# esulimma/LONER

Measured on AMD Instinct MI355X. Metric: ray-samples/sec per optimizer step; rendered-depth L1 vs reference, higher is better.
Workload: dtype fp16 params/activations, fp32 accumulate+optimizer; 1 GPU; C2: 16 KF x (512 + 0 sky) rays x 512 samples per GPU, L=16 T=2^18 hash grid + 64-wide sigma MLP, default loss (L1_JS); rays_per_gpu=8192, samples_per_ray=512, global_rays=8192, parallelism=single, optimizer=replicated, launch=HIP graph replay (one graph per window and OGM-or-not step), field_state=trained: the steps below follow 384 untimed pre-training steps (config.pretrain), poses=fixed (ground-truth poses, use_gt_poses: the north-star driver)

## Files before the change

### include/loner_amd.h

```cpp
#ifndef LONER_AMD_H
#define LONER_AMD_H

#include <stdint.h>

#ifdef __cplusplus
extern "C" {
#endif

#define LNR_OK 0
#define LNR_ERR_ARG (-1)
#define LNR_ERR_HIP (-2)

#define LNR_MAX_LEVELS 32

const char* lnr_last_error(void);
int lnr_version(void);

typedef struct lnr_step_scalars {
  uint32_t key;
  float los_lambda;
  float los_eps;
  float adam_step_size;
  float adam_bc2_sqrt;
  uint32_t pad[3];
// ... 147 lines not shown

int lnr_composite(const float* rays, const float* z, const float* sigma, int64_t n_rays, int32_t n_samples,
                  int32_t strategy, float noise_std, const float* noise, uint32_t key, int64_t ray_offset,
                  float* weights, float* depth, float* opacity, float* variance, void* stream);
int lnr_composite_loss_bwd(const float* rays, const float* z, const float* sigma, const float* depth_gt,
                           int64_t n_rays, int32_t n_samples, float noise_std, const float* noise, uint32_t key,
                           int64_t ray_offset, const lnr_loss_params* lp, float* weights, float* depth,
                           float* opacity, float* d_sigma, float* ray_stats, void* stream);
int lnr_composite_bwd(const float* rays, const float* z, const float* sigma, int64_t n_rays, int32_t n_samples,
                      int32_t strategy, float noise_std, const float* noise, uint32_t key, int64_t ray_offset,
                      const float* g_weights, const float* g_depth, const float* g_opacity, const float* g_variance,
                      float* d_sigma, float* d_ray, void* stream);
int64_t lnr_field_train_workspace_words(int64_t n_rays, int32_t n_samples);
int lnr_field_train(const uint16_t* w, const uint32_t* enc, int64_t enc_stride, const float* rays, const float* z,
                    const float* depth_gt, int64_t n_rays, int32_t n_samples, float noise_std, const float* noise,
                    uint32_t key, int64_t ray_offset, const lnr_loss_params* lp, float* d_enc, float* d_w,
                    float* workspace, float* ray_stats, float* depth, float* opacity, float* weights,
                    float* d_enc_level_max, uint32_t* d_enc_jac, void* stream);
int lnr_field_sigma_phase(const uint16_t* w, const uint32_t* enc, int64_t enc_stride, const float* rays,
                          const float* z, int64_t n_rays, int32_t n_samples, int32_t lo, int32_t hi, float noise_std,
                          const float* noise, uint32_t key, int64_t ray_offset, const lnr_loss_params* lp,
                          float* workspace, const uint32_t* list_in, const uint32_t* count_in, uint32_t* list_out,
                          uint32_t* count_out, double* transmittance, void* scratch, void* stream);
int lnr_pose_grad(const float* rays, const float* z, const float* d_pos, const float* d_ray, int64_t n_rays,
                  int32_t n_samples, const int64_t* slots, int64_t slot0, const int32_t* slot_kf, const float* slot_pose,
                  const float* pose6, int32_t n_kf, float scale, float far_range, float* ray_ws, float* grad,
                  void* stream);
int lnr_pose_adam(float* pose6, float* m, float* v, const float* grad, const uint8_t* optimise, int32_t n_kf,
                  int64_t step, float lr, float beta1, float beta2, float eps, float* rows, void* stream);
int lnr_field_render(const uint16_t* w, const uint32_t* enc, int64_t enc_stride, const float* rays, const float* z,
                     int64_t n_rays, int32_t n_samples, int32_t strategy, float noise_std, const float* noise,
                     uint32_t key, int64_t ray_offset, float* depth, float* opacity, float* variance,
                     float* weights, void* stream);
int lnr_rgb_render(const uint16_t* w_rgb, int32_t n_hidden_layers, const uint32_t* enc_rgb, int64_t enc_stride,
                   const float* rays, const float* weights, int64_t n_rays, int32_t n_samples, float* rgb,
                   void* stream);
int lnr_loss_finalize(const float* ray_stats, int64_t n_rays, const lnr_loss_params* lp, float* out, void* stream);

int lnr_count_opaque(const float* depth_gt, int64_t n_rays, float far_ref, const float* dev_far_ref, float* out,
                     void* stream);

#define LNR_SELECT_RANDOM 0
#define LNR_SELECT_MASK 1
#define LNR_SELECT_ALL 2
#define LNR_SELECT_GIVEN 3

// ... 113 lines not shown
```

### loner_amd/_lib.py

```python
import ctypes
import os

import torch

LIB_PATH = os.path.join(os.path.dirname(os.path.abspath(__file__)), "_lib", "libloner_amd.so")
LIB_PATH = os.environ.get("LONER_AMD_LIB", LIB_PATH)
MAX_LEVELS = 32
RAY_STATS = 5
SIGMA_MLP_PARAMS = 64 * 32 + 16 * 64

LOSS_KINDS = {"L1_JS": 0, "L2_JS": 1, "L1_LOS": 2, "L2_LOS": 3}
RENDER_STRATEGIES = {"default": 0, "adjusted": 1}
BWD_COUNTS_READY = 1
BWD_NO_ACCUM = 2
BWD_LEVEL_MAX_READY = 4
BWD_LIVE = 8
BWD_PREPARE_ONLY = 16
BWD_PREPARED = 32

c_p = ctypes.c_void_p
c_i64 = ctypes.c_int64
c_i32 = ctypes.c_int32
c_u32 = ctypes.c_uint32
c_f = ctypes.c_float
# ... 21 lines not shown
ADAM_MAX_RANGES = 8


class AdamEpilogue(ctypes.Structure):
    _fields_ = [("param", ctypes.c_void_p), ("shadow", ctypes.c_void_p), ("m", ctypes.c_void_p), ("v", ctypes.c_void_p),
                ("step", ctypes.c_int32), ("lr", ctypes.c_double), ("beta1", ctypes.c_double),
                ("beta2", ctypes.c_double), ("eps", ctypes.c_double), ("dev_step", ctypes.c_void_p)]


class LossParams(ctypes.Structure):
    _fields_ = [("kind", ctypes.c_int32), ("scale", ctypes.c_float), ("los_lambda", ctypes.c_float),
                ("depthloss_lambda", ctypes.c_float), ("min_depth_eps", ctypes.c_float),
                ("min_js", ctypes.c_float), ("max_js", ctypes.c_float), ("js_alpha", ctypes.c_float),
                ("los_eps", ctypes.c_float), ("far_ref", ctypes.c_float), ("inv_n_opaque", ctypes.c_float),
                ("inv_rs", ctypes.c_float), ("dev_n_opaque", ctypes.c_void_p), ("dev_far_ref", ctypes.c_void_p),
                ("dev_status", ctypes.c_void_p), ("dev_loss_out", ctypes.c_void_p), ("flags", ctypes.c_int32),
                ("dev_step", ctypes.c_void_p), ("dev_d_ray", ctypes.c_void_p), ("dev_term_hist", ctypes.c_void_p)]


LP_DW_OVERWRITE = 1
LP_SIGMA_READY = 2
LP_FORWARD_ONLY = 4
LP_BACKWARD_ONLY = 8


STATUS_NAN_LOSS, STATUS_INF_LOSS, STATUS_SIGMA_CLIPPED, STATUS_NONFINITE_OUTPUT = 1, 2, 4, 8


SELECT = {"RANDOM": 0, "MASK": 1, "ALL": 2, "GIVEN": 3}


class RayWindowDesc(ctypes.Structure):
    _fields_ = [("n_kf", ctypes.c_int32), ("scale", ctypes.c_float), ("shift", ctypes.c_float * 3),
                ("r_min", ctypes.c_float), ("r_max", ctypes.c_float), ("poses", c_p), ("dirs", c_p), ("dists", c_p),
                ("scan_off", c_p), ("order", c_p), ("n_trunk", c_p), ("sky_dirs", c_p), ("sky_off", c_p),
                ("ray_off", c_p), ("n_sel", c_p), ("n_sel_trunk", c_p), ("dev_step", c_p)]


class MotionComp(ctypes.Structure):
    _fields_ = [("start_rot", ctypes.c_float * 9), ("start_t", ctypes.c_float * 3), ("delta_t", ctypes.c_float * 3),
                ("axis", ctypes.c_float * 3), ("angle", ctypes.c_float), ("t0", ctypes.c_float), ("t1", ctypes.c_float),
                ("target_inv", ctypes.c_float * 12), ("identity", ctypes.c_int32)]


class CameraDesc(ctypes.Structure):
    _fields_ = [("width", ctypes.c_int32), ("height", ctypes.c_int32), ("channels", ctypes.c_int32),
# ... 34 lines not shown
    "lnr_hashgrid_bwd_rays_atomic": (ctypes.c_int, [ctypes.POINTER(GridDesc), c_p, c_p, c_i64, c_i32, c_p, c_i64, c_p,
                                                    c_p]),
    "lnr_enc_to_aos": (ctypes.c_int, [c_p, c_i64, c_i64, c_u32, c_p, c_p]),
    "lnr_aos_grad_to_enc": (ctypes.c_int, [c_p, c_p, c_i64, c_u32, c_p, c_i64, c_p]),
    "lnr_sh_encode": (ctypes.c_int, [c_p, c_i64, c_i32, c_p, c_p]),
    "lnr_sigma_mlp_fwd": (ctypes.c_int, [c_p, c_p, c_i64, c_i64, c_p, c_p]),
    "lnr_dw_workspace_words": (c_i64, [c_i64]),
    "lnr_field_train_workspace_words": (c_i64, [c_i64, c_i32]),
    "lnr_sigma_mlp_bwd": (ctypes.c_int, [c_p, c_p, c_i64, c_i64, c_p, c_p, c_p, c_p, c_p]),
    "lnr_step_key": (c_u32, [c_u32, c_u32]),
    "lnr_sample_ogm": (ctypes.c_int, [c_p, c_i64, c_i32, c_p, c_i32, c_f, c_p, c_p, c_u32, c_i64, c_p, c_p, c_p]),
    "lnr_sample_uniform": (ctypes.c_int, [c_p, c_i64, c_i32, c_f, c_p, c_u32, c_i64, c_p, c_p, c_p]),
    "lnr_composite": (ctypes.c_int, [c_p, c_p, c_p, c_i64, c_i32, c_i32, c_f, c_p, c_u32, c_i64, c_p, c_p, c_p, c_p,
                                     c_p]),
    "lnr_composite_bwd": (ctypes.c_int, [c_p, c_p, c_p, c_i64, c_i32, c_i32, c_f, c_p, c_u32, c_i64, c_p, c_p, c_p,
                                         c_p, c_p, c_p, c_p]),
    "lnr_composite_loss_bwd": (ctypes.c_int, [c_p, c_p, c_p, c_p, c_i64, c_i32, c_f, c_p, c_u32, c_i64,
                                              ctypes.POINTER(LossParams), c_p, c_p, c_p, c_p, c_p, c_p]),
    "lnr_field_train": (ctypes.c_int, [c_p, c_p, c_i64, c_p, c_p, c_p, c_i64, c_i32, c_f, c_p, c_u32, c_i64,
                                       ctypes.POINTER(LossParams), c_p, c_p, c_p, c_p, c_p, c_p, c_p, c_p, c_p,
                                       c_p]),
    "lnr_field_sigma_phase": (ctypes.c_int, [c_p, c_p, c_i64, c_p, c_p, c_i64, c_i32, c_i32, c_i32, c_f, c_p, c_u32,
                                             c_i64, ctypes.POINTER(LossParams), c_p, c_p, c_p, c_p, c_p, c_p, c_p, c_p]),
    "lnr_pose_grad": (ctypes.c_int, [c_p, c_p, c_p, c_p, c_i64, c_i32, c_p, c_i64, c_p, c_p, c_p, c_i32, c_f, c_f, c_p,
                                     c_p, c_p]),
    "lnr_pose_adam": (ctypes.c_int, [c_p, c_p, c_p, c_p, c_p, c_i32, c_i64, c_f, c_f, c_f, c_f, c_p, c_p]),
    "lnr_field_render": (ctypes.c_int, [c_p, c_p, c_i64, c_p, c_p, c_i64, c_i32, c_i32, c_f, c_p, c_u32, c_i64, c_p,
                                        c_p, c_p, c_p, c_p]),
    "lnr_rgb_render": (ctypes.c_int, [c_p, c_i32, c_p, c_i64, c_p, c_p, c_i64, c_i32, c_p, c_p]),
    "lnr_hashgrid_fwd_rays_phase": (ctypes.c_int, [ctypes.POINTER(GridDesc), c_p, c_p, c_i64, c_i32, c_p, c_p, c_i64,
                                                   c_p, c_i64, c_p, c_p, c_i64, c_i32, c_i32, c_p]),
    "lnr_hashgrid_fwd_rays_live": (ctypes.c_int, [ctypes.POINTER(GridDesc), c_p, c_p, c_i64, c_i32, c_p, c_p, c_p, c_i64,
                                                  c_p]),
    "lnr_hashgrid_fwd_rays_live_ws": (ctypes.c_int, [ctypes.POINTER(GridDesc), c_p, c_p, c_i64, c_i32, c_p, c_p, c_p,
                                                     c_i64, c_p, c_i64, c_p]),
    "lnr_hashgrid_bwd_rays_live": (ctypes.c_int, [ctypes.POINTER(GridDesc), c_p, c_p, c_i64, c_i32, c_p, c_i64, c_p, c_p,
                                                  c_p, c_i64, c_i32, c_p]),
    "lnr_status_scan": (ctypes.c_int, [c_p, c_i64, c_u32, c_p, c_p]),
    "lnr_rgb_mlp_params": (c_i64, [c_i32]),
    "lnr_rgb_train_workspace_bytes": (c_i64, [c_i32, c_i64]),
    "lnr_rgb_train": (ctypes.c_int, [c_p, c_i32, c_p, c_i64, c_p, c_p, c_p, c_i64, c_i32, c_f, c_p, c_p, c_p, c_p,
                                     c_p, c_i64, c_p, c_p]),
    "lnr_build_camera_rays": (ctypes.c_int, [ctypes.POINTER(CameraDesc), c_p, c_p, c_p, c_i64, c_p, c_p, c_p]),
    "lnr_build_camera_rays_window": (ctypes.c_int, [c_p, c_i32, c_p, c_p, c_i64, c_i64, c_i64, c_p, c_p, c_p]),
    "lnr_motion_compensate": (ctypes.c_int, [ctypes.POINTER(MotionComp), c_p, c_p, c_p, c_i64, c_p]),
    "lnr_sky_rays_capacity": (c_i64, []),
# ... 83 lines not shown
```

### loner_amd/csrc/field.hip

```cpp
#include "common.hpp"
#include "mlp.hpp"

namespace lnr {

constexpr int NT = 256;
constexpr int NW = NT / 64;

enum SigmaSrc { kSigmaGiven = 0, kSigmaMLP = 1 };

struct FieldArgs {
  const float* rays;
  const float* z;
  const float* sigma_in;
  const uint16_t* w;
  const uint32_t* enc;
  int64_t enc_stride;
  const float* depth_gt;
  const float* noise;
  int64_t n_rays;
  int32_t S;
  float noise_std;
  uint32_t key;
  int64_t ray_offset;
  lnr_loss_params lp;
// ... 845 lines not shown
#pragma unroll
    for (int j = 0; j < kErtCompactPer; ++j) mine += r[j] != ~0u ? 1u : 0u;
    uint32_t inc = mine;
#pragma unroll
    for (int o = 1; o < 64; o <<= 1) {
      const uint32_t v = __shfl_up(inc, o, 64);
      if (lane >= o) inc += v;
    }
    if (lane == 63) wsum[wid] = inc;
    __syncthreads();
    uint32_t off = base + inc - mine, tot = 0;
    for (int w = 0; w < kErtCompactThreads / 64; ++w) {
      const uint32_t v = wsum[w];
      if (w < wid) off += v;
      tot += v;
    }
#pragma unroll
    for (int j = 0; j < kErtCompactPer; ++j)
      if (r[j] != ~0u) list_out[off++] = r[j];
    base += tot;
    __syncthreads();
  }
  if (t == 0) count_out[0] = base;
}

template <int C>
__global__ void __launch_bounds__(NT) k_composite_wave(FieldArgs a) {
  if (a.denc_max && blockIdx.x == 0 && threadIdx.x < kSigmaLevels) a.denc_max[threadIdx.x] = 0.f;
  extern __shared__ __attribute__((aligned(16))) char smem[];
  const int lane = threadIdx.x & 63, wid = threadIdx.x >> 6;
  constexpr int S = 64 * C;
  float* sig = reinterpret_cast<float*>(smem) + wid * S;
  for (int64_t r = (int64_t)blockIdx.x * kWavesPerBlock + wid; r < a.n_rays; r += (int64_t)gridDim.x * kWavesPerBlock) {
#pragma unroll
    for (int k = 0; k < C; ++k) sig[64 * k + lane] = a.d_sigma[r * S + 64 * k + lane];
    wave_lds_handoff();
    composite_loss_wave<C>(a, sig, r);
    wave_lds_handoff();
#pragma unroll
    for (int k = 0; k < C; ++k) a.d_sigma[r * S + 64 * k + lane] = sig[64 * k + lane];
    wave_lds_handoff();
  }
}

template <class T>
__device__ __forceinline__ T ld_off(const T* base, uint32_t byte_off) {
// ... 687 lines not shown
  LNR_REQUIRE(n_rays < (int64_t(1) << 31), "lnr_field_sigma_phase: too many rays");
  if (n_rays == 0) return LNR_OK;
  LNR_REQUIRE(w && enc && workspace && (lo == 0 || (list_in && count_in)) && (!list_in || count_in),
              "lnr_field_sigma_phase: null pointer (a phase after the first needs the list of rays still alive)");
  LNR_REQUIRE(hi == n_samples || (list_out && count_out && transmittance && scratch),
              "lnr_field_sigma_phase: null pointer (the phase's transmittance update)");
  FieldArgs a{};
  a.w = w; a.enc = enc; a.enc_stride = enc_stride; a.rays = rays; a.z = z; a.n_rays = n_rays; a.S = n_samples;
  a.noise_std = noise_std; a.noise = noise; a.key = key; a.ray_offset = ray_offset;
  if (lp) a.lp = *lp;
  a.d_sigma = workspace + lnr_dw_workspace_words(n_rays);
  hipStream_t st = as_stream(stream);
  const uint32_t* lin = lo == 0 ? nullptr : list_in;
  const uint32_t* cin = lo == 0 ? nullptr : count_in;
  uint32_t* keep = reinterpret_cast<uint32_t*>(scratch);
  const int64_t want = (n_rays + kWavesPerBlock - 1) / kWavesPerBlock;
  hipLaunchKernelGGL(k_sigma_phase, dim3((unsigned)(want < 8192 ? want : 8192)), dim3(NT), 0, st, a, lin, cin, lo, hi,
                     transmittance, keep, kErtTMin);
  if (hi < n_samples)
    hipLaunchKernelGGL(k_ert_compact, dim3(1), dim3(kErtCompactThreads), 0, st, keep, cin, n_rays, list_out, count_out);
  LNR_RETURN_LAUNCH("lnr_field_sigma_phase");
}

extern "C" int lnr_field_render(const uint16_t* w, const uint32_t* enc, int64_t enc_stride, const float* rays,
                                const float* z, int64_t n_rays, int32_t n_samples, int32_t strategy, float noise_std,
                                const float* noise, uint32_t key, int64_t ray_offset, float* depth, float* opacity,
                                float* variance, float* weights, void* stream) {
  if (int e = check_rays(rays, z, n_rays, n_samples, "lnr_field_render")) return e;
  LNR_REQUIRE(strategy == LNR_RENDER_DEFAULT || strategy == LNR_RENDER_ADJUSTED,
              "Unknown render strategy: %d", strategy);
  LNR_REQUIRE(n_samples % 64 == 0, "lnr_field_render: n_samples=%d must be a multiple of 64", n_samples);
  LNR_REQUIRE(enc_stride >= n_rays * (int64_t)n_samples, "lnr_field_render: enc_stride too small");
  if (n_rays == 0) return LNR_OK;
  LNR_REQUIRE(w && enc && depth, "lnr_field_render: null pointer");
  FieldArgs a{};
  a.w = w; a.enc = enc; a.enc_stride = enc_stride; a.rays = rays; a.z = z; a.n_rays = n_rays; a.S = n_samples;
  a.noise_std = noise_std; a.noise = noise; a.key = key; a.ray_offset = ray_offset;
  a.depth = depth; a.opacity = opacity; a.variance = variance; a.weights = weights;
  const int nb = field_blocks(n_rays);
#if LNR_FIELD_SPLIT
  if (weights) {
    hipStream_t st = as_stream(stream);
    a.d_sigma = weights;
    const int64_t units = n_rays * (int64_t)n_samples / kSigmaFwdUnit;
    const int64_t wantu = (units + kWavesPerBlock - 1) / kWavesPerBlock;
    hipLaunchKernelGGL(k_sigma_fwd_tiles, dim3((int)(wantu < 8192 ? wantu : 8192)), dim3(NT), 0, st, a);
// ... 38 lines not shown
```

### loner_amd/csrc/hashgrid.hip

```cpp
#include "hashgrid.hpp"

namespace lnr {

__device__ __forceinline__ void store_enc(uint32_t* p, uint32_t v) { __builtin_nontemporal_store(v, p); }

__device__ __forceinline__ void fine_gather(const uint32_t* __restrict__ tl, const FineCell& c, uint32_t (&v)[8]) {
#pragma unroll
  for (int j = 0; j < 4; ++j) {
    v[2 * j] = tl[c.e[j]];
    v[2 * j + 1] = tl[c.e[j] ^ c.d];
  }
}

#ifndef LNR_ENC_PAIRED
#define LNR_ENC_PAIRED true
#endif
__device__ __forceinline__ uint32_t dpp_pair_swap(uint32_t v) {
  return (uint32_t)__builtin_amdgcn_update_dpp(0, (int)v, 0xB1, 0xF, 0xF, false);
}
__device__ __forceinline__ void fine_gather_paired(const uint32_t* __restrict__ tl, const FineCell& c, bool use,
                                                   uint32_t (&v)[8]) {
  const bool odd = (threadIdx.x & 1) != 0;
  const uint32_t pd = dpp_pair_swap(c.d);
  const bool puse = dpp_pair_swap(use ? 1u : 0u) != 0u;
  const uint32_t d_even = odd ? pd : c.d, d_odd = odd ? c.d : pd;
  const bool use_even = odd ? puse : use, use_odd = odd ? use : puse;
  uint32_t s0[4], s1[4];
#pragma unroll
  for (int j = 0; j < 4; ++j) {
    const uint32_t pe = dpp_pair_swap(c.e[j]);
    const uint32_t e_even = odd ? pe : c.e[j], e_odd = odd ? c.e[j] : pe;
    const uint32_t a0 = odd ? (e_even ^ d_even) : e_even;
    const uint32_t a1 = odd ? (e_odd ^ d_odd) : e_odd;
    s0[j] = use_even ? tl[a0] : 0u;
    s1[j] = use_odd ? tl[a1] : 0u;
  }
#pragma unroll
  for (int j = 0; j < 4; ++j) {
    const uint32_t r = dpp_pair_swap(odd ? s0[j] : s1[j]);
    v[2 * j] = odd ? r : s0[j];
    v[2 * j + 1] = odd ? s1[j] : r;
  }
}

#ifndef LNR_ENC_SPT2_MIN_N
#define LNR_ENC_SPT2_MIN_N (1 << 18)
#endif

#ifndef LNR_ENC_LPB
#define LNR_ENC_LPB 4
#endif
#ifndef LNR_ENC_GROUP_MIN_ROWS
#define LNR_ENC_GROUP_MIN_ROWS 512
#endif
#ifndef LNR_ENC_GROUP4_MIN_ROWS
#define LNR_ENC_GROUP4_MIN_ROWS 2048
#endif
inline int enc_levels_per_group(const lnr_grid_desc* d, int64_t n_sb) {
  if (n_sb < LNR_ENC_GROUP_MIN_ROWS) return 1;
  const int64_t level_bytes = (int64_t)4 << d->log2_hashmap_size;
  for (int g = LNR_ENC_LPB; g > 1; g /= 2)
    if (d->n_levels % g == 0 && g * level_bytes <= ((int64_t)4 << 20) && (g < 4 || n_sb >= LNR_ENC_GROUP4_MIN_ROWS))
      return g;
  return 1;
// ... 467 lines not shown
```

### loner_amd/csrc/hashgrid.hpp

```cpp
#pragma once
#include "common.hpp"
#include <cstdlib>

namespace lnr {

struct LevelParams {
  float scale;
  uint32_t res;
  uint32_t size;
  uint32_t size_mask;
  uint32_t offset;
  uint32_t hashed;
  uint32_t fine;
};

constexpr int kChunkLog2 = 12;
constexpr int kChunk = 1 << kChunkLog2;
constexpr int kMaxChunksPerLevel = 128;
constexpr int kMaxBuckets = 2048;
constexpr int kAccumGroups = 512;
constexpr int kMaxUnits = kMaxBuckets + kAccumGroups;
struct UnitTable {
  uint32_t n_units, n_cut, pad0, pad1;
  uint2 unit[kMaxUnits];
// ... 210 lines not shown
__device__ __forceinline__ void fine_cell(const LevelParams& p, float x, float y, float z, FineCell& c) {
  const float px = fmaf(p.scale, x, 0.5f), py = fmaf(p.scale, y, 0.5f), pz = fmaf(p.scale, z, 0.5f);
  const float fx = floorf(px), fy = floorf(py), fz = floorf(pz);
  const uint32_t cx = (uint32_t)(int)fx, cy = (uint32_t)(int)fy, cz = (uint32_t)(int)fz;
  c.tx = px - fx;
  c.ty = py - fy;
  c.tz = pz - fz;
  const uint32_t hy0 = cy * 2654435761u, hy1 = (cy + 1u) * 2654435761u;
  const uint32_t hz0 = cz * 805459861u, hz1 = (cz + 1u) * 805459861u;
  const uint32_t m = p.size_mask;
  c.e[0] = (cx ^ hy0 ^ hz0) & m;
  c.e[1] = (cx ^ hy1 ^ hz0) & m;
  c.e[2] = (cx ^ hy0 ^ hz1) & m;
  c.e[3] = (cx ^ hy1 ^ hz1) & m;
  c.d = (cx ^ (cx + 1u)) & m;
}
__device__ __forceinline__ float fine_weight(const FineCell& c, int j, int bx) {
  float w = bx ? c.tx : 1.0f - c.tx;
  w *= (j & 1) ? c.ty : 1.0f - c.ty;
  w *= (j & 2) ? c.tz : 1.0f - c.tz;
  return w;
}

struct RunInfo {
  unsigned long long heads;
  int head_lane;
  bool tail;
};
__device__ __forceinline__ RunInfo lane_runs(uint32_t key) {
  const int lane = threadIdx.x & 63;
  const uint32_t prev = __shfl_up(key, 1, 64);
  const bool head = (lane == 0) || (prev != key);
  RunInfo ri;
  ri.heads = __ballot(head);
  ri.head_lane = 63 - __clzll(ri.heads & ((2ull << lane) - 1ull));
  ri.tail = (lane == 63) || ((ri.heads >> (lane + 1)) & 1ull);
  return ri;
}
__device__ __forceinline__ void run_sum(const RunInfo& ri, float& v0, float& v1) {
  const int lane = threadIdx.x & 63;
#pragma unroll
  for (int o = 1; o < 64; o <<= 1) {
    const float q0 = __shfl_up(v0, o, 64), q1 = __shfl_up(v1, o, 64);
    if (lane - o >= ri.head_lane) {
      v0 += q0;
      v1 += q1;
// ... 308 lines not shown
```

### loner_amd/step.py

```python
import math
import os
import warnings
from dataclasses import dataclass, field

import torch

from . import _lib as L


@dataclass
class LossConfig:
    loss_selection: str = "L1_JS"
    min_js_score: float = 1.0
    max_js_score: float = 10.0
    js_alpha: float = 1.0
    decay_los_lambda: bool = False
    los_lambda: float = 1000.0
    min_los_lambda: float = 10.0
    los_lambda_decay_rate: float = 0.001
    los_lambda_decay_steps: float = 15000
    decay_depth_eps: bool = True
    depth_eps: float = 3.0
    min_depth_eps: float = 0.5
    depth_eps_decay_rate: float = 0.95
# ... 99 lines not shown
    @property
    def grad_mlp(self):
        return self.grad[:self.n_mlp]

    def state_dict(self):
        return {"params": self.params[:self.n_params].clone(), "occupancy_grid": self.occ.clone(),
                "adam_step": self.adam_step, "m": self.m[:self.n_params].clone(), "v": self.v[:self.n_params].clone()}

    def load_state_dict(self, sd):
        self.params[:self.n_params].copy_(sd["params"])
        self.occ.copy_(sd["occupancy_grid"].reshape(-1))
        if "m" in sd:
            self.m[:self.n_params].copy_(sd["m"])
            self.v[:self.n_params].copy_(sd["v"])
            self.adam_step = int(sd.get("adam_step", 0))
        self.refresh_shadow()


FUSED_ADAM_MAX_N = 1 << 17
AR_CUT_DEFAULT = 6
AR_CUT_TWO_GROUPS = 8

ERT_SAMPLE_NS, ERT_FIXED_US, ERT_PHASE_US = 0.150, 5.0, 28.0
TERM_HIST_SLOTS = 256
ERT_MAX_CUTS = 4
ERT_MARGIN = 0.02


def ert_alive(hist, S):
    import numpy as np
    h = np.asarray(hist, dtype=np.float64)
    tot = h.sum()
    if tot <= 0:
        return np.ones(S // 64 + 1)
    tail = np.cumsum(h[::-1])[::-1]
    return tail / tot


def ert_cost_us(bounds, alive, S, n_samples):
    full = ERT_SAMPLE_NS * 1e-3 * n_samples
    if bounds is None:
        return full
    t = ERT_FIXED_US + ERT_PHASE_US * (len(bounds) - 2)
    for lo, hi in zip(bounds[:-1], bounds[1:]):
        t += full * float(alive[lo // 64]) * (hi - lo) / S
    return t


def ert_plan(hist, S, n_samples, current=None, max_cuts=ERT_MAX_CUTS, margin=ERT_MARGIN):
    import itertools
    if S % 64 or S < 128:
        return None
    alive = ert_alive(hist, S)
    full = ert_cost_us(None, alive, S, n_samples)
    pos = list(range(64, S, 64))
    best, best_t = None, full
    for k in range(1, min(max_cuts, len(pos)) + 1):
        for cuts in itertools.combinations(pos, k):
            b = [0, *cuts, S]
            t = ert_cost_us(b, alive, S, n_samples)
            if t < best_t:
                best, best_t = b, t
    cur_t = ert_cost_us(current, alive, S, n_samples)
    return best if best_t < cur_t - margin * full else current


class StepEngine:

    def __init__(self, state: FieldState, n_rays: int, seed: int = 0, allreduce=None, ray_offset: int = 0,
                 count_in_forward: bool = True, zero=None, reduce_scatter=None, all_gather=None, ar_cut=None):
        self.state = state
        self.cfg = state.cfg
        self.n_rays = n_rays
        self.S = self.cfg.n_samples
        self.N = n_rays * self.S
        self.seed = seed
        self.ray_offset = ray_offset
        self.count_in_forward = count_in_forward
        self.lr_factor = 1.0
        self.status = torch.zeros(1, dtype=torch.int32, device=state.device)
        self._warned_clip = False
        nl = self.cfg.n_levels
        nbk = int(os.environ.get("LONER_AR_BUCKETS", "2"))
        if nbk <= 1:
            cuts = [nl, 0]
        elif nbk == 2:
# ... 65 lines not shown
        self.fused_adam = {"0": False, "1": True}.get(os.environ.get("LONER_FUSED_ADAM", "auto"), "auto")
        self._pp, self._pp_parity = None, 0
        self._pp_stream = torch.cuda.Stream(device=dev)
        self._pp_fork = torch.cuda.Event()
        g = os.environ.get("LONER_GRAPH", "auto")
        self.use_graph = (g == "1") or (g == "auto" and (self.N <= (1 << 18) or self.N >= (1 << 22)))
        self._dev_steps = torch.zeros(8, dtype=torch.int32, device=dev)
        self.dev_step = self._dev_steps
        self._dev_step = None
        self._graphs, self._graph_window = {}, None
        self._capture_stream = torch.cuda.Stream(device=dev)
        self.live_bwd = {"0": False, "1": True}.get(os.environ.get("LONER_LIVE_BWD", "auto"), "auto")
        self.live_on, self.live_off, self.live_probe_every = 0.25, 0.15, 16
        self._live = self.live_bwd is True
        self._probe_ev, self._probe_ctr, self._probe_n = None, self.live_probe_every, 1
        self._probe_host = torch.zeros(1, dtype=torch.int64).pin_memory() if torch.cuda.is_available() else None
        self.pose_grad = False
        self.map_frozen = False
        self.poses = None
        self.d_ray = self.d_pos = None
        self._last_batch = None
        self.ert = {"0": False, "1": True}.get(os.environ.get("LONER_ERT", "auto"), "auto")
        self.ert_cuts = [float(v) for v in os.environ.get("LONER_ERT_CUTS", "0.5,0.625,0.75").split(",") if v.strip()]
        self.ert_lists = torch.zeros(2, max(n_rays, 1), dtype=torch.int32, device=dev)
        self.ert_counts = torch.zeros(2, dtype=torch.int32, device=dev)
        self.ert_T = torch.ones(n_rays, dtype=torch.float64, device=dev)
        self.ert_keep = torch.zeros(max(n_rays, 1), dtype=torch.int32, device=dev)
        self._ert_est = None
        self._ert_last = None
        self._ert_plan = None
        self._ert_next = None
        nb = self.S // 64 + 1
        self.term_hist = (torch.zeros(TERM_HIST_SLOTS, nb, dtype=torch.int32, device=dev) if self.S % 64 == 0
                          else None)
        pin = torch.cuda.is_available() and self.term_hist is not None
        self._term_host = torch.zeros(TERM_HIST_SLOTS, nb, dtype=torch.int32).pin_memory() if pin else None
        self._term_prev = [0] * (self.S // 64 + 1)
        self._term_ev, self._term_ctr = None, self.live_probe_every
        self._pp_bufs = [dict(rays=self.rays if i == 0 else torch.empty_like(self.rays),
                              dgt=self.depth_gt if i == 0 else torch.empty_like(self.depth_gt),
                              valid=self.ray_valid if i == 0 else torch.empty_like(self.ray_valid),
                              far=self.far_ref if i == 0 else torch.empty_like(self.far_ref),
                              z=self.z if i == 0 else torch.empty_like(self.z))
                         for i in range(2)]

    def ert_bounds(self):
        S = self.S
        if not self.compact_denc or S % 64 or self.ert is False:
            return None
        if self.ert == "auto":
            return None if self._ert_plan is None else list(self._ert_plan)
        b = sorted({int(round(f * S / 64)) * 64 for f in self.ert_cuts if 0.0 < f < 1.0} - {0, S})
        return [0] + b + [S] if b else None

    def _mlp_adam(self, dsp, s):
        st = self.state
        nm, nt = st.n_mlp, 2 * st.n_entries
        L.call("lnr_adam_step", st.params[:nm], st.shadow[:nm], st.grad[:nm], st.m[:nm], st.v[:nm], nm,
               st.adam_step, self.map_lr(), 0.9, 0.999, 1e-8, dsp, s)
        if st.n_padded > nm + nt:
            o = nm + nt
            L.call("lnr_adam_step", st.params[o:], st.shadow[o:], st.grad[o:], st.m[o:], st.v[o:], st.n_padded - o,
                   st.adam_step, self.map_lr(), 0.9, 0.999, 1e-8, dsp, s)

    def fuses_adam(self, N=None):
        N = self.N if N is None else N
        return self.allreduce is None and self.zero is None and self.compact_denc and (
            self.fused_adam is True or (self.fused_adam == "auto" and (N <= FUSED_ADAM_MAX_N or self._live)))

    def ert_alive_last(self):
        b = self._ert_last
        if b is None or len(b) < 3:
            return 1.0
        return int(self.ert_counts[(len(b) - 3) % 2].item()) / max(self._r_last, 1)

    def _ert_key(self):
        b = self.ert_bounds()
        return None if b is None else tuple(b)

    def ert_probe(self):
        if self.ert != "auto" or self._term_host is None:
            return
        ev = self._term_ev
        if ev is not None and ev.query():
            cur = [int(v) & 0xFFFFFFFF for v in self._term_host.long().sum(0).tolist()]
            d = [(c - p) & 0xFFFFFFFF for c, p in zip(cur, self._term_prev)]
            self._term_prev = cur
            self._term_ev = None
            if sum(d) > 0:
                defer = self._ert_est is not None and self._graph_window is not None
                plan = ert_plan(d, self.S, self._r_last * self.S, self._ert_plan,
                                margin=0.0 if defer else ERT_MARGIN)
                if plan != self._ert_plan or self._ert_est is None:
                    nxt = (plan, [float(v) for v in ert_alive(d, self.S)])
                    if defer:
                        self._ert_next = nxt
                    else:
                        self._ert_plan, self._ert_est = nxt
                        self._ert_next = None
                else:
                    self._ert_next = None
        self._term_ctr += 1
        if self._term_ev is None and self._term_ctr >= self.live_probe_every:
            self._term_ctr = 0
            self._term_host.copy_(self.term_hist, non_blocking=True)
            self._term_ev = torch.cuda.Event()
            self._term_ev.record()

    def map_lr(self):
        return 0.0 if self.map_frozen else self.cfg.lr * self.lr_factor

    def set_poses(self, poses):
        self.poses = poses
        self.pose_grad = poses is not None
        if self.pose_grad and self.d_ray is None:
# ... 91 lines not shown
        else:
            L.call("lnr_count_opaque", depth_gt, R, 0.0 if far_h is None else far_h, dev_far, self.n_opaque, s)
        lp = self.loss_params(global_step, iteration_idx, scale, far_h, n_glob, dev_far)
        dsp = None if dev_step is None else dev_step.data_ptr()
        lp.dev_step = dsp
        lp.dev_d_ray = self.d_ray.data_ptr() if self.pose_grad else None
        lp.dev_term_hist = self.term_hist.data_ptr() if self.ert is not False and self.term_hist is not None else None
        self._dev_step = dsp
        self._apply_pending_ogm()
        m(prof, "sample")
        if presampled:
            pass
        elif cfg.sampler == "OGM":
            L.call("lnr_sample_ogm", rays, R, S, st.occ, cfg.occ_res, cfg.perturb, u_jitter, u_pdf, key,
                   self.ray_offset, self.z, dsp, s)
        else:
            L.call("lnr_sample_uniform", rays, R, S, cfg.perturb, u_jitter, key, self.ray_offset, self.z, dsp, s)
        m(prof, "sample")
        self.finish()
        m(prof, "encode")
        fwd_hist = self.count_in_forward and not self._live
        ert = self.ert_bounds()
        self._ert_last = ert
        if ert is not None:
            lp.flags |= L.LP_SIGMA_READY
            for q in range(len(ert) - 1):
                lo, hi = ert[q], ert[q + 1]
                hist = q == 0 and fwd_hist
                lin = None if q == 0 else self.ert_lists[(q - 1) % 2]
                cin = None if q == 0 else self.ert_counts[(q - 1) % 2:(q - 1) % 2 + 1]
                est = self._ert_est
                expect = 0 if (q == 0 or est is None) else int(est[lo // 64] * R) + 64
                L.call("lnr_hashgrid_fwd_rays_phase", L.ctypes.byref(st.desc), rays, self.z, R, S, st.table_f16,
                       self.enc, N, self.bwd_ws if hist else None, self.bwd_ws_bytes if hist else 0, lin, cin,
                       expect, lo, hi, s)
                m(prof, "sigma_phase")
                L.call("lnr_field_sigma_phase", st.mlp_f16, self.enc, N, rays, self.z, R, S, lo, hi,
                       cfg.raw_noise_std, noise, key, self.ray_offset, L.ctypes.byref(lp), self.ws, lin, cin,
                       self.ert_lists[q % 2], self.ert_counts[q % 2:q % 2 + 1], self.ert_T, self.ert_keep, s)
                m(prof, "sigma_phase")
        elif fwd_hist:
            L.call("lnr_hashgrid_fwd_rays", L.ctypes.byref(st.desc), rays, self.z, R, S, st.table_f16, self.enc, N,
                   self.bwd_ws, self.bwd_ws_bytes, s)
        else:
            L.call("lnr_hashgrid_fwd_rays", L.ctypes.byref(st.desc), rays, self.z, R, S, st.table_f16, self.enc, N,
                   None, 0, s)
        m(prof, "encode")
        if fork_count or self.allreduce is not None:
            main.wait_event(self._join)
        if pending is not None:
            pending.wait()
        flags = (L.BWD_COUNTS_READY if fwd_hist else 0) | L.BWD_LEVEL_MAX_READY | (
            L.BWD_LIVE if self._live else 0)
        split = (self.split_bwd and self._live and self.compact_denc and prof is None and self.allreduce is None
                 and self.zero is None and S in (64, 128, 256, 512))
        mlp_adam_done = False

        def field_train(extra):
            lp.flags |= extra
            L.call("lnr_field_train", st.mlp_f16, self.enc, N, rays, self.z, depth_gt, R, S, cfg.raw_noise_std, noise,
                   key, self.ray_offset, L.ctypes.byref(lp), self.d_enc, st.grad_mlp, self.ws, self.stats, self.depth,
                   self.opacity, None, self.level_max_ptr, self.d_jac if self.compact_denc else None, s)
            lp.flags &= ~extra
# ... 408 lines not shown
```

Before: 4.940 billion ray-samples/s.

## Add fused per-ray ERT march kernel for fine-grained early ray termination tail

Adds a kernel that, for rays still alive after the last coarse ERT phase, marches 64-sample units one at a time. Each step does the hash-grid encode, sigma MLP and transmittance update in one block per ray, and exits once transmittance drops below a threshold, zero-filling the remaining sigma. The ERT planner gains candidate plans whose tail runs as 64-sample march steps, with a cost model for them, and the feature is on by default. The aim is to skip encode and MLP work on terminated samples at finer granularity and with fewer launches than the phase-list kernels. The cost is one block per ray with serial per-unit barriers, lower parallelism on the tail, and more complex planner logic.

```diff
diff --git a/include/loner_amd.h b/include/loner_amd.h
--- a/include/loner_amd.h
+++ b/include/loner_amd.h
@@ -193,6 +193,11 @@
                           const float* noise, uint32_t key, int64_t ray_offset, const lnr_loss_params* lp,
                           float* workspace, const uint32_t* list_in, const uint32_t* count_in, uint32_t* list_out,
                           uint32_t* count_out, double* transmittance, void* scratch, void* stream);
+int lnr_field_ert_march(const lnr_grid_desc* d, const uint16_t* table, uint32_t* enc, int64_t enc_stride,
+                        const uint16_t* w, const float* rays, const float* z, int64_t n_rays, int32_t n_samples,
+                        int32_t lo, float noise_std, const float* noise, uint32_t key, int64_t ray_offset,
+                        const lnr_loss_params* lp, float* workspace, const uint32_t* list_in,
+                        const uint32_t* count_in, double* transmittance, void* stream);
 int lnr_pose_grad(const float* rays, const float* z, const float* d_pos, const float* d_ray, int64_t n_rays,
                   int32_t n_samples, const int64_t* slots, int64_t slot0, const int32_t* slot_kf, const float* slot_pose,
                   const float* pose6, int32_t n_kf, float scale, float far_range, float* ray_ws, float* grad,
diff --git a/loner_amd/_lib.py b/loner_amd/_lib.py
--- a/loner_amd/_lib.py
+++ b/loner_amd/_lib.py
@@ -67,6 +67,7 @@
 LP_SIGMA_READY = 2
 LP_FORWARD_ONLY = 4
 LP_BACKWARD_ONLY = 8
+ERT_T_MIN = 1e-50
 
 
 STATUS_NAN_LOSS, STATUS_INF_LOSS, STATUS_SIGMA_CLIPPED, STATUS_NONFINITE_OUTPUT = 1, 2, 4, 8
@@ -147,6 +148,9 @@
                                        c_p]),
     "lnr_field_sigma_phase": (ctypes.c_int, [c_p, c_p, c_i64, c_p, c_p, c_i64, c_i32, c_i32, c_i32, c_f, c_p, c_u32,
                                              c_i64, ctypes.POINTER(LossParams), c_p, c_p, c_p, c_p, c_p, c_p, c_p, c_p]),
+    "lnr_field_ert_march": (ctypes.c_int, [ctypes.POINTER(GridDesc), c_p, c_p, c_i64, c_p, c_p, c_p, c_i64, c_i32, c_i32,
+                                           c_f, c_p, c_u32, c_i64, ctypes.POINTER(LossParams), c_p, c_p, c_p, c_p,
+                                           c_p]),
     "lnr_pose_grad": (ctypes.c_int, [c_p, c_p, c_p, c_p, c_i64, c_i32, c_p, c_i64, c_p, c_p, c_p, c_i32, c_f, c_f, c_p,
                                      c_p, c_p]),
     "lnr_pose_adam": (ctypes.c_int, [c_p, c_p, c_p, c_p, c_p, c_i32, c_i64, c_f, c_f, c_f, c_f, c_p, c_p]),
diff --git a/loner_amd/csrc/field.hip b/loner_amd/csrc/field.hip
--- a/loner_amd/csrc/field.hip
+++ b/loner_amd/csrc/field.hip
@@ -1,4 +1,5 @@
 #include "common.hpp"
+#include "hashgrid.hpp"
 #include "mlp.hpp"
 
 namespace lnr {
@@ -891,6 +892,125 @@
     __syncthreads();
   }
   if (t == 0) count_out[0] = base;
+}
+
+struct MarchLevels {
+  LevelParams lv[kSigmaLevels];
+};
+constexpr int kMarchPitch = 68;
+#ifndef LNR_MARCH_WAVES
+#define LNR_MARCH_WAVES 8
+#endif
+struct MarchWeightsLds {
+  const half8_t* p;
+  __device__ __forceinline__ half8_t A0(int t) const { return p[t * 64 + (threadIdx.x & 63)]; }
+  __device__ __forceinline__ float w1(int k) const { return (float)p[(4 + (k >> 3)) * 64 + (threadIdx.x & 63)][k & 7]; }
+  __device__ __forceinline__ void stage(half8_t* lds, const SigmaWeights& sw) {
+    const int lane = threadIdx.x & 63;
+    if (threadIdx.x < 64) {
+#pragma unroll
+      for (int t = 0; t < 4; ++t) lds[t * 64 + lane] = sw.a0[t];
+      lds[4 * 64 + lane] = sw.w1h[0];
+      lds[5 * 64 + lane] = sw.w1h[1];
+    }
+    p = lds;
+  }
+};
+__global__ void __launch_bounds__(NT) __attribute__((amdgpu_waves_per_eu(LNR_MARCH_WAVES)))
+k_ert_march(FieldArgs a, MarchLevels ml, const uint32_t* __restrict__ table, uint32_t* __restrict__ enc,
+            const uint32_t* __restrict__ list, const uint32_t* __restrict__ count, int32_t lo,
+            double* __restrict__ trans, double t_min) {
+  if (blockIdx.x >= count[0]) return;
+  __shared__ uint32_t encb[kSigmaLevels * kMarchPitch];
+  __shared__ float sigb[kSigmaFwdUnit];
+  const int lane = threadIdx.x & 63, c = lane & 15, g = lane >> 4;
+  const int wid = __builtin_amdgcn_readfirstlane((int)(threadIdx.x >> 6));
+  const int S = a.S;
+  const int64_t r = (int64_t)list[blockIdx.x];
+  const float* ry = a.rays + 13 * r;
+  const PosFromRays pos{a.rays, a.z, S};
+  const PosFromRays::Raw ray{ry[0], ry[1], ry[2], ry[3], ry[4], ry[5], 0.f};
+  const float dnorm = sqrtf(ray.dx * ray.dx + ray.dy * ray.dy + ray.dz * ray.dz);
+  const float* zr = a.z + r * S;
+  const uint32_t gr = (uint32_t)(a.ray_offset + r);
+  __shared__ half8_t wlds[6 * 64];
+  MarchWeightsLds sw;
+  {
+    SigmaWeights sr;
+    load_sigma_weights(a.w, sr);
+    sw.stage(wlds, sr);
+  }
+  double t = trans[r];
+  bool clipped = false;
+  for (int u0 = lo; u0 < S; u0 += kSigmaFwdUnit) {
+    const int i = u0 + lane;
+    const int64_t n = r * S + i;
+    const float zi = zr[i];
+    PosFromRays::Raw q = ray;
+    q.t = zi;
+    float x, y, z;
+    pos.eval(q, x, y, z);
+    for (int k = 0; k < kSigmaLevels / NW; ++k) {
+      const int l = wid + NW * k;
+      const LevelParams& lv = ml.lv[l];
+      uint32_t word;
+      if (lv.fine) {
+        FineCell fc;
+        uint32_t v[8];
+        fine_cell(lv, x, y, z, fc);
+        fine_gather_paired(table + lv.offset, fc, true, v);
+        word = enc_blend_fine(fc, v);
+      } else {
+        Corners cn;
+        uint32_t v[8];
+        level_corners(lv, x, y, z, cn);
+#pragma unroll
+        for (int j = 0; j < 8; ++j) v[j] = table[cn.idx[j]];
+        word = enc_blend(cn, v);
+      }
+      store_enc(enc + (int64_t)l * a.enc_stride + n, word);
+      encb[l * kMarchPitch + lane] = word;
+    }
+    lds_barrier();
+    half8_t b;
+#pragma unroll
+    for (int j = 0; j < 4; ++j) {
+      const uint32_t v = encb[(4 * g + j) * kMarchPitch + 16 * wid + c];
+      b[2 * j + 0] = __builtin_bit_cast(_Float16, (uint16_t)(v & 0xFFFFu));
+      b[2 * j + 1] = __builtin_bit_cast(_Float16, (uint16_t)(v >> 16));
+    }
+    SigmaHidden h;
+    const float sgm = sigma_tile_fwd(sw, b, h);
+    const float sg16 = sigma_to_f16(sgm);
+    if (g == 0) {
+      a.d_sigma[r * S + u0 + 16 * wid + c] = sg16;
+      sigb[16 * wid + c] = sg16;
+    }
+    clipped |= !isfinite(round_f16(sgm));
+    if (u0 + kSigmaFwdUnit >= S) break;
+    lds_barrier();
+    {
+      const float mine = sigb[lane];
+      const float dl = (i + 1 < S) ? (zr[i + 1] - zi) : 1e10f;
+      const float delta = dl * dnorm;
+      float nz = 0.f;
+      if (a.noise) nz = a.noise[n] * a.noise_std;
+      else if (a.noise_std > 0.f) nz = rand_normal(step_key_of(a), kStreamNoise, gr, (uint32_t)i) * a.noise_std;
+      const float sr = fmaxf(mine + nz, 0.f);
+      const float alpha = 1.0f - expf(-(delta * sr));
+      double P = 1.0;
+      P *= (double)((1.0f - alpha) + 1e-10f);
+#pragma unroll
+      for (int o = 32; o > 0; o >>= 1) P *= __shfl_xor(P, o, 64);
+      t = t * P;
+    }
+    if (threadIdx.x == 0) trans[r] = t;
+    if (!(t >= t_min)) {
+      for (int j = u0 + kSigmaFwdUnit + (int)threadIdx.x; j < S; j += NT) a.d_sigma[r * S + j] = 0.f;
+      break;
+    }
+  }
+  if (a.lp.dev_status && __any(clipped) && lane == 0) atomicOr(a.lp.dev_status, LNR_STATUS_SIGMA_CLIPPED);
 }
 
 template <int C>
@@ -1624,6 +1744,37 @@
   LNR_RETURN_LAUNCH("lnr_field_sigma_phase");
 }
 
+extern "C" int lnr_field_ert_march(const lnr_grid_desc* d, const uint16_t* table, uint32_t* enc, int64_t enc_stride,
+                                   const uint16_t* w, const float* rays, const float* z, int64_t n_rays,
+                                   int32_t n_samples, int32_t lo, float noise_std, const float* noise, uint32_t key,
+                                   int64_t ray_offset, const lnr_loss_params* lp, float* workspace,
+                                   const uint32_t* list_in, const uint32_t* count_in, double* transmittance,
+                                   void* stream) {
+  if (int e = check_rays(rays, z, n_rays, n_samples, "lnr_field_ert_march")) return e;
+  LNR_REQUIRE(d != nullptr && d->n_levels == (uint32_t)kSigmaLevels && d->n_features == 2,
+              "lnr_field_ert_march: the sigma grid has %d levels of 2 features", kSigmaLevels);
+  LNR_REQUIRE(n_samples % 64 == 0 && lo > 0 && lo < n_samples && lo % 64 == 0,
+              "lnr_field_ert_march: the march from %d of %d samples must start and end on whole 64-sample waves", lo,
+              n_samples);
+  LNR_REQUIRE(enc_stride >= n_rays * (int64_t)n_samples && enc_stride < (int64_t(1) << 26),
+              "lnr_field_ert_march: bad enc_stride");
+  LNR_REQUIRE(n_rays < (int64_t(1) << 31), "lnr_field_ert_march: too many rays");
+  if (n_rays == 0) return LNR_OK;
+  LNR_REQUIRE(table && enc && w && workspace && list_in && count_in && transmittance,
+              "lnr_field_ert_march: null pointer");
+  FieldArgs a{};
+  a.w = w; a.enc = enc; a.enc_stride = enc_stride; a.rays = rays; a.z = z; a.n_rays = n_rays; a.S = n_samples;
+  a.noise_std = noise_std; a.noise = noise; a.key = key; a.ray_offset = ray_offset;
+  if (lp) a.lp = *lp;
+  a.d_sigma = workspace + lnr_dw_workspace_words(n_rays);
+  const GridArgs ga = make_args(d, n_samples);
+  MarchLevels ml;
+  for (int l = 0; l < kSigmaLevels; ++l) ml.lv[l] = ga.lv[l];
+  hipLaunchKernelGGL(k_ert_march, dim3((unsigned)n_rays), dim3(NT), 0, as_stream(stream), a, ml,
+                     reinterpret_cast<const uint32_t*>(table), enc, list_in, count_in, lo, transmittance, kErtTMin);
+  LNR_RETURN_LAUNCH("lnr_field_ert_march");
+}
+
 extern "C" int lnr_field_render(const uint16_t* w, const uint32_t* enc, int64_t enc_stride, const float* rays,
                                 const float* z, int64_t n_rays, int32_t n_samples, int32_t strategy, float noise_std,
                                 const float* noise, uint32_t key, int64_t ray_offset, float* depth, float* opacity,
diff --git a/loner_amd/csrc/hashgrid.hip b/loner_amd/csrc/hashgrid.hip
--- a/loner_amd/csrc/hashgrid.hip
+++ b/loner_amd/csrc/hashgrid.hip
@@ -1,45 +1,12 @@
 #include "hashgrid.hpp"
 
 namespace lnr {
-
-__device__ __forceinline__ void store_enc(uint32_t* p, uint32_t v) { __builtin_nontemporal_store(v, p); }
 
 __device__ __forceinline__ void fine_gather(const uint32_t* __restrict__ tl, const FineCell& c, uint32_t (&v)[8]) {
 #pragma unroll
   for (int j = 0; j < 4; ++j) {
     v[2 * j] = tl[c.e[j]];
     v[2 * j + 1] = tl[c.e[j] ^ c.d];
-  }
-}
-
-#ifndef LNR_ENC_PAIRED
-#define LNR_ENC_PAIRED true
-#endif
-__device__ __forceinline__ uint32_t dpp_pair_swap(uint32_t v) {
-  return (uint32_t)__builtin_amdgcn_update_dpp(0, (int)v, 0xB1, 0xF, 0xF, false);
-}
-__device__ __forceinline__ void fine_gather_paired(const uint32_t* __restrict__ tl, const FineCell& c, bool use,
-                                                   uint32_t (&v)[8]) {
-  const bool odd = (threadIdx.x & 1) != 0;
-  const uint32_t pd = dpp_pair_swap(c.d);
-  const bool puse = dpp_pair_swap(use ? 1u : 0u) != 0u;
-  const uint32_t d_even = odd ? pd : c.d, d_odd = odd ? c.d : pd;
-  const bool use_even = odd ? puse : use, use_odd = odd ? use : puse;
-  uint32_t s0[4], s1[4];
-#pragma unroll
-  for (int j = 0; j < 4; ++j) {
-    const uint32_t pe = dpp_pair_swap(c.e[j]);
-    const uint32_t e_even = odd ? pe : c.e[j], e_odd = odd ? c.e[j] : pe;
-    const uint32_t a0 = odd ? (e_even ^ d_even) : e_even;
-    const uint32_t a1 = odd ? (e_odd ^ d_odd) : e_odd;
-    s0[j] = use_even ? tl[a0] : 0u;
-    s1[j] = use_odd ? tl[a1] : 0u;
-  }
-#pragma unroll
-  for (int j = 0; j < 4; ++j) {
-    const uint32_t r = dpp_pair_swap(odd ? s0[j] : s1[j]);
-    v[2 * j] = odd ? r : s0[j];
-    v[2 * j + 1] = odd ? s1[j] : r;
   }
 }
 
diff --git a/loner_amd/csrc/hashgrid.hpp b/loner_amd/csrc/hashgrid.hpp
--- a/loner_amd/csrc/hashgrid.hpp
+++ b/loner_amd/csrc/hashgrid.hpp
@@ -256,6 +256,72 @@
   return w;
 }
 
+__device__ __forceinline__ void store_enc(uint32_t* p, uint32_t v) { __builtin_nontemporal_store(v, p); }
+
+#ifndef LNR_ENC_PAIRED
+#define LNR_ENC_PAIRED true
+#endif
+__device__ __forceinline__ uint32_t dpp_pair_swap(uint32_t v) {
+  return (uint32_t)__builtin_amdgcn_update_dpp(0, (int)v, 0xB1, 0xF, 0xF, false);
+}
+__device__ __forceinline__ void fine_gather_paired(const uint32_t* __restrict__ tl, const FineCell& c, bool use,
+                                                   uint32_t (&v)[8]) {
+  const bool odd = (threadIdx.x & 1) != 0;
+  const uint32_t pd = dpp_pair_swap(c.d);
+  const bool puse = dpp_pair_swap(use ? 1u : 0u) != 0u;
+  const uint32_t d_even = odd ? pd : c.d, d_odd = odd ? c.d : pd;
+  const bool use_even = odd ? puse : use, use_odd = odd ? use : puse;
+  uint32_t s0[4], s1[4];
+#pragma unroll
+  for (int j = 0; j < 4; ++j) {
+    const uint32_t pe = dpp_pair_swap(c.e[j]);
+    const uint32_t e_even = odd ? pe : c.e[j], e_odd = odd ? c.e[j] : pe;
+    const uint32_t a0 = odd ? (e_even ^ d_even) : e_even;
+    const uint32_t a1 = odd ? (e_odd ^ d_odd) : e_odd;
+    s0[j] = use_even ? tl[a0] : 0u;
+    s1[j] = use_odd ? tl[a1] : 0u;
+  }
+#pragma unroll
+  for (int j = 0; j < 4; ++j) {
+    const uint32_t r = dpp_pair_swap(odd ? s0[j] : s1[j]);
+    v[2 * j] = odd ? r : s0[j];
+    v[2 * j + 1] = odd ? s1[j] : r;
+  }
+}
+
+__device__ __forceinline__ void enc_blend_keep_scalar(float& f0, float& f1) {
+  asm("" : "+v"(f0));
+  asm("" : "+v"(f1));
+}
+__device__ __forceinline__ uint32_t enc_blend_pack(float f0, float f1) {
+  uint32_t w = (uint32_t)f2h(f0) | ((uint32_t)f2h(f1) << 16);
+  asm("" : "+v"(w));
+  return w;
+}
+__device__ __forceinline__ uint32_t enc_blend_fine(const FineCell& c, const uint32_t (&v)[8]) {
+  float f0 = 0.f, f1 = 0.f;
+#pragma unroll
+  for (int k = 0; k < 8; ++k) {
+    const float w = fine_weight(c, k >> 1, k & 1);
+    const float2 t = half2_to_float2(v[k]);
+    f0 = fmaf(w, t.x, f0);
+    f1 = fmaf(w, t.y, f1);
+    if (k < 7) enc_blend_keep_scalar(f0, f1);
+  }
+  return enc_blend_pack(f0, f1);
+}
+__device__ __forceinline__ uint32_t enc_blend(const Corners& c, const uint32_t (&v)[8]) {
+  float f0 = 0.f, f1 = 0.f;
+#pragma unroll
+  for (int k = 0; k < 8; ++k) {
+    const float2 t = half2_to_float2(v[k]);
+    f0 = fmaf(c.w[k], t.x, f0);
+    f1 = fmaf(c.w[k], t.y, f1);
+    if (k < 7) enc_blend_keep_scalar(f0, f1);
+  }
+  return enc_blend_pack(f0, f1);
+}
+
 struct RunInfo {
   unsigned long long heads;
   int head_lane;
diff --git a/loner_amd/step.py b/loner_amd/step.py
--- a/loner_amd/step.py
+++ b/loner_amd/step.py
@@ -145,6 +145,8 @@
 AR_CUT_TWO_GROUPS = 8
 
 ERT_SAMPLE_NS, ERT_FIXED_US, ERT_PHASE_US = 0.150, 5.0, 28.0
+ERT_MARCH_SAMPLE_NS, ERT_MARCH_FIXED_US = 0.278, 27.0
+ERT_MARCH = os.environ.get("LONER_ERT_MARCH", "1") != "0"
 TERM_HIST_SLOTS = 256
 ERT_MAX_CUTS = 4
 ERT_MARGIN = 0.02
@@ -160,31 +162,48 @@
     return tail / tot
 
 
-def ert_cost_us(bounds, alive, S, n_samples):
+def ert_march_start(bounds):
+    if bounds is None:
+        return None
+    i = len(bounds) - 1
+    while i > 1 and bounds[i] - bounds[i - 1] == 64:
+        i -= 1
+    return i if len(bounds) - 1 - i >= 2 else None
+
+
+def ert_cost_us(bounds, alive, S, n_samples, march=None):
     full = ERT_SAMPLE_NS * 1e-3 * n_samples
     if bounds is None:
         return full
-    t = ERT_FIXED_US + ERT_PHASE_US * (len(bounds) - 2)
-    for lo, hi in zip(bounds[:-1], bounds[1:]):
+    i0 = ert_march_start(bounds) if (ERT_MARCH if march is None else march) else None
+    n_ph = len(bounds) - 1 if i0 is None else i0
+    t = ERT_FIXED_US + ERT_PHASE_US * (n_ph - 1)
+    for lo, hi in zip(bounds[:n_ph], bounds[1:n_ph + 1]):
         t += full * float(alive[lo // 64]) * (hi - lo) / S
+    if i0 is not None:
+        t += ERT_MARCH_FIXED_US
+        for lo in bounds[i0:-1]:
+            t += ERT_MARCH_SAMPLE_NS * 1e-3 * n_samples * float(alive[lo // 64]) * 64 / S
     return t
 
 
-def ert_plan(hist, S, n_samples, current=None, max_cuts=ERT_MAX_CUTS, margin=ERT_MARGIN):
+def ert_plan(hist, S, n_samples, current=None, max_cuts=ERT_MAX_CUTS, margin=ERT_MARGIN, march=None):
     import itertools
     if S % 64 or S < 128:
         return None
+    march = ERT_MARCH if march is None else march
     alive = ert_alive(hist, S)
-    full = ert_cost_us(None, alive, S, n_samples)
+    full = ert_cost_us(None, alive, S, n_samples, march)
     pos = list(range(64, S, 64))
     best, best_t = None, full
-    for k in range(1, min(max_cuts, len(pos)) + 1):
-        for cuts in itertools.combinations(pos, k):
-            b = [0, *cuts, S]
-            t = ert_cost_us(b, alive, S, n_samples)
-            if t < best_t:
-                best, best_t = b, t
-    cur_t = ert_cost_us(current, alive, S, n_samples)
+    cands = [[0, *cuts, S] for k in range(1, min(max_cuts, len(pos)) + 1) for cuts in itertools.combinations(pos, k)]
+    if march:
+        cands += [[0, *range(c1, S + 1, 64)] for c1 in pos[:-1]]
+    for b in cands:
+        t = ert_cost_us(b, alive, S, n_samples, march)
+        if t < best_t:
+            best, best_t = b, t
+    cur_t = ert_cost_us(current, alive, S, n_samples, march)
     return best if best_t < cur_t - margin * full else current
 
 
@@ -296,12 +315,14 @@
         self._last_batch = None
         self.ert = {"0": False, "1": True}.get(os.environ.get("LONER_ERT", "auto"), "auto")
         self.ert_cuts = [float(v) for v in os.environ.get("LONER_ERT_CUTS", "0.5,0.625,0.75").split(",") if v.strip()]
+        self.ert_march = ERT_MARCH
         self.ert_lists = torch.zeros(2, max(n_rays, 1), dtype=torch.int32, device=dev)
         self.ert_counts = torch.zeros(2, dtype=torch.int32, device=dev)
         self.ert_T = torch.ones(n_rays, dtype=torch.float64, device=dev)
         self.ert_keep = torch.zeros(max(n_rays, 1), dtype=torch.int32, device=dev)
         self._ert_est = None
         self._ert_last = None
+        self._ert_marched = None
         self._ert_plan = None
         self._ert_next = None
         nb = self.S // 64 + 1
@@ -346,11 +367,13 @@
         b = self._ert_last
         if b is None or len(b) < 3:
             return 1.0
+        if self._ert_marched is not None:
+            return int((self.ert_T[:self._r_last] >= L.ERT_T_MIN).sum().item()) / max(self._r_last, 1)
         return int(self.ert_counts[(len(b) - 3) % 2].item()) / max(self._r_last, 1)
 
     def _ert_key(self):
         b = self.ert_bounds()
-        return None if b is None else tuple(b)
+        return None if b is None else (tuple(b), bool(self.ert_march))
 
     def ert_probe(self):
         if self.ert != "auto" or self._term_host is None:
@@ -364,7 +387,7 @@
             if sum(d) > 0:
                 defer = self._ert_est is not None and self._graph_window is not None
                 plan = ert_plan(d, self.S, self._r_last * self.S, self._ert_plan,
-                                margin=0.0 if defer else ERT_MARGIN)
+                                margin=0.0 if defer else ERT_MARGIN, march=self.ert_march)
                 if plan != self._ert_plan or self._ert_est is None:
                     nxt = (plan, [float(v) for v in ert_alive(d, self.S)])
                     if defer:
@@ -502,9 +525,12 @@
         fwd_hist = self.count_in_forward and not self._live
         ert = self.ert_bounds()
         self._ert_last = ert
+        i0 = ert_march_start(ert) if self.ert_march else None
+        self._ert_marched = i0
         if ert is not None:
             lp.flags |= L.LP_SIGMA_READY
-            for q in range(len(ert) - 1):
+            mp = prof if i0 is None else None
+            for q in range(len(ert) - 1 if i0 is None else i0):
                 lo, hi = ert[q], ert[q + 1]
                 hist = q == 0 and fwd_hist
                 lin = None if q == 0 else self.ert_lists[(q - 1) % 2]
@@ -514,11 +540,16 @@
                 L.call("lnr_hashgrid_fwd_rays_phase", L.ctypes.byref(st.desc), rays, self.z, R, S, st.table_f16,
                        self.enc, N, self.bwd_ws if hist else None, self.bwd_ws_bytes if hist else 0, lin, cin,
                        expect, lo, hi, s)
-                m(prof, "sigma_phase")
+                m(mp, "sigma_phase")
                 L.call("lnr_field_sigma_phase", st.mlp_f16, self.enc, N, rays, self.z, R, S, lo, hi,
                        cfg.raw_noise_std, noise, key, self.ray_offset, L.ctypes.byref(lp), self.ws, lin, cin,
                        self.ert_lists[q % 2], self.ert_counts[q % 2:q % 2 + 1], self.ert_T, self.ert_keep, s)
-                m(prof, "sigma_phase")
+                m(mp, "sigma_phase")
+            if i0 is not None:
+                q = i0 - 1
+                L.call("lnr_field_ert_march", L.ctypes.byref(st.desc), st.table_f16, self.enc, N, st.mlp_f16, rays,
+                       self.z, R, S, ert[i0], cfg.raw_noise_std, noise, key, self.ray_offset, L.ctypes.byref(lp),
+                       self.ws, self.ert_lists[q % 2], self.ert_counts[q % 2:q % 2 + 1], self.ert_T, s)
         elif fwd_hist:
             L.call("lnr_hashgrid_fwd_rays", L.ctypes.byref(st.desc), rays, self.z, R, S, st.table_f16, self.enc, N,
                    self.bwd_ws, self.bwd_ws_bytes, s)
```

Measured after the change: 5.001 billion ray-samples/s (median of 6 runs). +1.2%, better.
